# YukeWang96/QGTC_PPoPP22

Hardware: AMD Instinct MI355X
Metric: effective bit-GEMM TOPS (2*M*K*N/t), 1-bit A x 1-bit X, M=K=4096, N=64 (higher is better)
Workload: dtype fp4 (E2M1 codes of bit planes on MFMA, exact f32 sums); 1 GPU; bitMM2Bit 4096x4096x64 a=1 w=1 ob=1 (BASELINE.json configs[1], 2_7c shape); inputs=seeded Bernoulli(0.5) adjacency, uniform w-bit features, packed, resident in HBM, parallelism=replica-per-GPU x1, no data-path collective, engine=auto, issue=eager

## Files before the change

### qgtc_ppopp22_amd/csrc/bitmm_fp4_stream.hip.h

```cpp
#pragma once

namespace {

constexpr int ST_WAVES = 8;
constexpr int ST_MUL = 4;
constexpr int ST_COLS = 64;
constexpr int ST_PITCH = 68;
constexpr int ST_PIECE = 1024;
constexpr int ST_GB = 64 * ST_MUL;
constexpr int ST_STAGES = 3;

constexpr int st_pieces(int rf, int cf) { return (32 * rf / 8 + 32 * cf / 8) * (ST_GB / 128); }
constexpr int st_lds_bytes(int rf, int cf) {
    const int stages = ST_STAGES * st_pieces(rf, cf) * ST_PIECE, part = ST_MUL * 4 * rf * cf * 1024, tile = 32 * rf * ST_PITCH * 4;
    return stages > part ? (stages > tile ? stages : tile) : (part > tile ? part : tile);
}

template <int RF, int CF>
__device__ __forceinline__ constexpr int st_exp_by(int n) {
    if constexpr (RF == 2 && CF == 1) { constexpr int t[] = {5, 6, 8, 9, 11, 12, 14, 15}; return t[n]; }
    else if constexpr (RF == 2 && CF == 2) { constexpr int t[] = {4, 5, 6, 7, 8, 9, 10, 11, 12, 13, 14, 15, 16, 17, 18, 19}; return t[n]; }
    else if constexpr (RF == 4 && CF == 1) { constexpr int t[] = {4, 5, 7, 8, 9, 10, 12, 13, 14, 15, 17, 18, 19, 20, 22, 23}; return t[n]; }
    else { constexpr int t[] = {4, 4, 5, 5, 6, 7, 8, 9, 10, 10, 11, 11, 12, 13, 14, 15, 16, 16, 17, 17, 18, 19, 20, 21, 22, 22, 23, 23, 24, 25, 26, 27}; return t[n]; }
}
template <int RF, int CF>
__device__ __forceinline__ constexpr int st_shift_by(int n) {
    if constexpr (RF == 2 && CF == 1) { constexpr int t[] = {0, 0, 0, 8, 12, 12, 12, 12}; return t[n]; }
    else if constexpr (RF == 2 && CF == 2) { constexpr int t[] = {0, 0, 0, 0, 0, 2, 4, 6, 8, 10, 12, 16, 16, 16, 16, 16}; return t[n]; }
    else if constexpr (RF == 4 && CF == 1) { constexpr int t[] = {0, 0, 0, 0, 0, 0, 0, 2, 4, 8, 12, 16, 20, 20, 20, 20}; return t[n]; }
    else { constexpr int t[] = {0, 0, 0, 0, 0, 0, 0, 0, 0, 0, 0, 0, 0, 2, 4, 6, 8, 14, 16, 20, 22, 24, 24, 24, 24, 24, 24, 24, 24, 24, 24, 24}; return t[n]; }
}

template <class F, int... I>
__device__ __forceinline__ void st_for_impl(F &&f, std::integer_sequence<int, I...>) { (f(std::integral_constant<int, I>{}), ...); }
template <int N, class F>
__device__ __forceinline__ void st_for(F &&f) { st_for_impl(f, std::make_integer_sequence<int, N>{}); }

__device__ __forceinline__ void st_dma(uint32_t lds_dst, uint32_t voff, i32x4 rsrc, uint32_t soff) {
    uint32_t keep;
    asm volatile("s_mov_b32 %0, m0\n\ts_mov_b32 m0, %1\n\ts_nop 0\n\tbuffer_load_dwordx4 %2, %3, %4 offen lds\n\ts_mov_b32 m0, %0"
                 : "=&s"(keep)
                 : "s"(lds_dst), "v"(voff), "s"(rsrc), "s"(soff)
                 : "memory");
}

template <int MODE, int RF, int CF>
__global__ __launch_bounds__(64 * ST_WAVES) void k_bitmm_fp4_stream(
    const uint32_t *__restrict__ Xp, const uint32_t *__restrict__ Wp, void *__restrict__ outp, uint32_t x_bytes, uint32_t w_bytes,
    uint32_t out_bytes, int M, int K, int N, int w_lines,
    uint32_t cfg , int n_wg) {
    static_assert((RF == 2 || RF == 4) && (CF == 1 || CF == 2), "32-line fragments of a multiplying wave: left, right");
    constexpr int TR = 32 * RF, WK = ST_MUL;
    constexpr int GB = ST_GB, BPG = GB / 128, GQ = GB / 16;
    constexpr int XP = (TR / 8) * BPG, WP = (32 * CF / 8) * BPG, TOT = XP + WP;
    constexpr int FW = ST_WAVES - ST_MUL;
    static_assert(XP % FW == 0 && TOT % FW == 0, "whole rounds of the fetching waves");
    constexpr int STAGE = TOT * ST_PIECE, STAGES = ST_STAGES;
    constexpr int DMAS = TOT / FW;
    static_assert(DMAS >= 1 && DMAS <= 31, "vmcnt immediate");
    extern __shared__ __attribute__((aligned(1024))) unsigned char st_lds[];
    int (*tile)[ST_PITCH] = reinterpret_cast<int (*)[ST_PITCH]>(st_lds);
    const int tid = threadIdx.x, lane = tid & 63;
    const int wv = __builtin_amdgcn_readfirstlane(tid >> 6);
    const int fl = lane & 31, hf = lane >> 5;
#ifdef QGTC_STAMPS
    unsigned long long st_[16] = {0, 0, 0, 0, 0, 0, 0, 0, 0, 0, 0, 0, 0, 0, 0, 0};
#define ST_STAMP(i) st_[i] = __builtin_amdgcn_s_memtime()
#else
#define ST_STAMP(i) do { } while (0)
#endif
    ST_STAMP(0);
#ifdef QGTC_STAMPS
    st_[13] = __builtin_amdgcn_s_memrealtime();
#endif
    const int ob = cfg & 255u, tiles_n = static_cast<int>(cfg >> 16);
    const bool zero_skip = ((cfg >> 8) & 1u) != 0u;
    int t = static_cast<int>(blockIdx.x);
    if (tiles_n > 1) t = xcd_consecutive(t, n_wg);
    const int tm = t / tiles_n, tn = t - tm * tiles_n;
    const int m0 = tm * TR, n0 = tn * ST_COLS;
    const int kq = step128(K);
    const uint32_t row_bytes = static_cast<uint32_t>(kq) * 16u;
    const uint32_t lds0 = static_cast<uint32_t>(reinterpret_cast<uintptr_t>(st_lds));
    (void)x_bytes; (void)w_bytes; (void)out_bytes; (void)w_lines;
    const int ng = (kq + GQ - 1) / GQ;
    constexpr int NQ = RF * CF * 4;
    f32x16 acc[RF][CF];

    if (wv >= ST_MUL) {
        const int fw = wv - ST_MUL;
        const i32x4 rs_x = {static_cast<int>(reinterpret_cast<uintptr_t>(Xp)), static_cast<int>((reinterpret_cast<uintptr_t>(Xp) >> 32) & 0xffffu), static_cast<int>(x_bytes), 0x00020000};
        const i32x4 rs_w = {static_cast<int>(reinterpret_cast<uintptr_t>(Wp)), static_cast<int>((reinterpret_cast<uintptr_t>(Wp) >> 32) & 0xffffu), static_cast<int>(w_bytes), 0x00020000};
        const int rr = lane >> 3, cc = lane & 7;
        const uint32_t swz = static_cast<uint32_t>(cc ^ (rr & 6)) * 16u;
#ifdef QGTC_STREAM_TUNE
        const uint32_t voff_x = static_cast<uint32_t>(((cfg >> 9) & 1u ? 0 : m0) + rr) * row_bytes + swz, voff_w = static_cast<uint32_t>(n0 + rr) * row_bytes + swz;
        const bool no_dma = ((cfg >> 10) & 1u) != 0u;
#else
        const uint32_t voff_x = static_cast<uint32_t>(m0 + rr) * row_bytes + swz, voff_w = static_cast<uint32_t>(n0 + rr) * row_bytes + swz;
        constexpr bool no_dma = false;
#endif
        auto issue = [&](int g) {
            if (g >= ng || no_dma) return;
            const uint32_t base = lds0 + static_cast<uint32_t>(g % STAGES) * STAGE;
            const uint32_t ko = static_cast<uint32_t>(g) * GB;
#pragma unroll
            for (int j = 0; j < DMAS; j++) {
                const int p = fw + FW * j;
                if (FW * j < XP) {
                    st_dma(base + static_cast<uint32_t>(p) * ST_PIECE, voff_x, rs_x, ko + static_cast<uint32_t>(8 * (p / BPG)) * row_bytes + 128u * (p % BPG));
                } else {
                    const int pw = p - XP;
                    st_dma(base + static_cast<uint32_t>(p) * ST_PIECE, voff_w, rs_w, ko + static_cast<uint32_t>(8 * (pw / BPG)) * row_bytes + 128u * (pw % BPG));
                }
            }
        };
        issue(0);
        issue(1);
        for (int g = 0; g < ng; g++) {
            if (g + 1 < ng) asm volatile("s_waitcnt vmcnt(%0)" ::"n"(DMAS) : "memory");
            else asm volatile("s_waitcnt vmcnt(0)" ::: "memory");
#ifdef QGTC_STAMPS
            if (g == 0) ST_STAMP(1); else if (g == 5) ST_STAMP(3); else if (g == 6) ST_STAMP(7);
#endif
            __builtin_amdgcn_s_barrier();
#ifdef QGTC_STAMPS
            if (g == 0) ST_STAMP(2); else if (g == 5) ST_STAMP(4); else if (g == 6) ST_STAMP(8);
#endif
            issue(g + 2);
        }
        ST_STAMP(11);
    } else {
        const int wk = wv;
        const uint32_t frag_off = static_cast<uint32_t>(fl & 7) * 128u + static_cast<uint32_t>((4 * (wk & 1) + hf) ^ (fl & 6)) * 16u + static_cast<uint32_t>(wk >> 1) * ST_PIECE;
        const uint32_t xa0 = static_cast<uint32_t>((fl >> 3) * BPG) * ST_PIECE + frag_off;
        const uint32_t wa0 = static_cast<uint32_t>(XP + (fl >> 3) * BPG) * ST_PIECE + frag_off;
        const int my_q = 8 * (wk >> 1) + 4 * (wk & 1) + hf;
#pragma unroll
        for (int i = 0; i < RF; i++)
#pragma unroll
            for (int j = 0; j < CF; j++)
#pragma unroll
                for (int r = 0; r < 16; r++) acc[i][j][r] = 0.0f;

        auto fetch = [&](auto tail, int g, int u, u32x4 (&xr)[RF], u32x4 (&wr)[CF]) {
            const unsigned char *stage = st_lds + (g % STAGES) * STAGE;
#pragma unroll
            for (int i = 0; i < RF; i++) xr[i] = *reinterpret_cast<const u32x4 *>(stage + ((xa0 + static_cast<uint32_t>(4 * i * BPG) * ST_PIECE) ^ (32u * u)));
#pragma unroll
            for (int j = 0; j < CF; j++) wr[j] = *reinterpret_cast<const u32x4 *>(stage + ((wa0 + static_cast<uint32_t>(4 * j * BPG) * ST_PIECE) ^ (32u * u)));
            if constexpr (decltype(tail)::value) {
                if (g == ng - 1 && g * GQ + my_q + 2 * u >= kq) {
#pragma unroll
                    for (int i = 0; i < RF; i++) xr[i] = u32x4{0u, 0u, 0u, 0u};
                }
            }
        };
        constexpr int MN = 4 * RF * CF, OPB = RF + CF, EN = 4 * OPB, EP = 3;
        i32x4 A[4], B[2][CF];
        auto expand = [&](auto e_, u32x4 (&xr)[RF], u32x4 (&wr)[CF]) {
            constexpr int e = decltype(e_)::value, s = e / OPB, o = e % OPB;
            constexpr uint32_t mask = s < 3 ? 0x11111111u << s : 0x11111111u;
            constexpr bool is_a = o == 0 || o > CF;
            constexpr int f = o == 0 ? 0 : (o > CF ? o - CF : o - 1);
            u32x4 v;
            if constexpr (is_a) v = xr[f]; else v = wr[f];
            const i32x4 r = {static_cast<int>(v.x & mask), static_cast<int>(v.y & mask), static_cast<int>(v.z & mask), static_cast<int>(v.w & mask)};
            if constexpr (is_a) { A[(s * RF + f) & 3] = r; asm volatile("" : "+v"(A[(s * RF + f) & 3])); }
            else { B[s & 1][f] = r; asm volatile("" : "+v"(B[s & 1][f])); }
        };
        auto shift = [&](auto z_, u32x4 (&xr)[RF], u32x4 (&wr)[CF]) {
            constexpr int z = decltype(z_)::value, o = z >> 2, el = z & 3;
            constexpr bool is_a = o == 0 || o > CF;
            constexpr int f = o == 0 ? 0 : (o > CF ? o - CF : o - 1);
            if constexpr (is_a) { xr[f][el] >>= 3; if constexpr (el == 3) asm volatile("" : "+v"(xr[f])); }
            else { wr[f][el] >>= 3; if constexpr (el == 3) asm volatile("" : "+v"(wr[f])); }
        };
        auto any_of = [&](const u32x4 (&xr)[RF]) {
            uint32_t any = 0u;
#pragma unroll
            for (int i = 0; i < RF; i++) any |= (xr[i].x | xr[i].y) | (xr[i].z | xr[i].w);
            return any;
        };
        auto skipped = [&](uint32_t any) { return zero_skip && __ballot(any != 0u) == 0ull; };
        auto first = [&](u32x4 (&xr)[RF], u32x4 (&wr)[CF]) {
            st_for<EP>([&](auto e_) { expand(e_, xr, wr); });
        };
        auto step = [&](auto with_next, u32x4 (&xr)[RF], u32x4 (&wr)[CF], u32x4 (&nx)[RF], u32x4 (&nw)[CF], uint32_t &any_next) {
            constexpr bool NEXT = decltype(with_next)::value;
            __builtin_amdgcn_sched_barrier(0);
            st_for<MN>([&](auto n_) {
                constexpr int n = decltype(n_)::value, s = n / (RF * CF), q = n % (RF * CF);
                constexpr int i = q / CF, j = (i & 1) ? CF - 1 - q % CF : q % CF;
                constexpr int sc = s < 3 ? 128 - s : 128;
                const i32x4 a4 = A[(s * RF + i) & 3], b4 = B[s & 1][j];
                const i32x8 a8 = __builtin_shufflevector(a4, a4, 0, 1, 2, 3, -1, -1, -1, -1);
                const i32x8 b8 = __builtin_shufflevector(b4, b4, 0, 1, 2, 3, -1, -1, -1, -1);
                acc[i][j] = __builtin_amdgcn_mfma_scale_f32_32x32x64_f8f6f4(a8, b8, acc[i][j], 4, 4, 0, sc, 0, sc);
                constexpr int e0 = n == 0 ? EP : st_exp_by<RF, CF>(n == 0 ? 0 : n - 1), e1 = st_exp_by<RF, CF>(n);
                st_for<e1 - e0>([&](auto k_) {
                    constexpr int e = e0 + decltype(k_)::value;
                    if constexpr (e < EN) expand(std::integral_constant<int, e>{}, xr, wr);
                    else if constexpr (NEXT) expand(std::integral_constant<int, e - EN>{}, nx, nw);
                });
                constexpr int z0 = n == 0 ? 0 : st_shift_by<RF, CF>(n == 0 ? 0 : n - 1), z1 = st_shift_by<RF, CF>(n);
                st_for<z1 - z0>([&](auto k_) { shift(std::integral_constant<int, z0 + decltype(k_)::value>{}, xr, wr); });
                if constexpr (NEXT && n == MN - 7) {
                    any_next = any_of(nx);
                    asm volatile("" : "+v"(any_next));
                }
                __builtin_amdgcn_sched_barrier(0);
            });
        };
        using with_next = std::integral_constant<bool, true>;
        using last_step = std::integral_constant<bool, false>;
        uint32_t any_now = 0u;
        auto multiply = [&](u32x4 (&xr)[RF], u32x4 (&wr)[CF], u32x4 (&nx)[RF], u32x4 (&nw)[CF]) {
            uint32_t any_next;
            if (skipped(any_now)) {
                first(nx, nw);
                any_next = any_of(nx);
            } else {
                step(with_next{}, xr, wr, nx, nw, any_next);
            }
            any_now = any_next;
        };
        u32x4 xp[RF], wp[CF], xq[RF], wq[CF];
        using any_group = std::integral_constant<bool, true>;
        using not_last = std::integral_constant<bool, false>;
        auto trip = [&](auto tail, int g) {
            fetch(tail, g, 1, xq, wq);
            multiply(xp, wp, xq, wq);
#ifdef QGTC_STAMPS
            if (g == 5) ST_STAMP(6); else if (g == 6) ST_STAMP(10);
#endif
            asm volatile("s_waitcnt lgkmcnt(0)" ::: "memory");
            __builtin_amdgcn_s_barrier();
#ifdef QGTC_STAMPS
            if (g == 4) ST_STAMP(4); else if (g == 5) ST_STAMP(8);
#endif
            fetch(tail, g + 1, 0, xp, wp);
            multiply(xq, wq, xp, wp);
        };
        __builtin_amdgcn_s_barrier();
        ST_STAMP(2);
        fetch(any_group{}, 0, 0, xp, wp);
        first(xp, wp);
        any_now = any_of(xp);
        int g = 0;
        for (; g + 2 < ng; g++) trip(not_last{}, g);
        for (; g + 1 < ng; g++) trip(any_group{}, g);
        fetch(any_group{}, g, 1, xq, wq);
        multiply(xp, wp, xq, wq);
        if (!skipped(any_now)) step(last_step{}, xq, wq, xp, wp, any_now);
#ifdef QGTC_STAMPS
        asm volatile("" : "+v"(acc[0][0]));
#endif
        ST_STAMP(11);
    }
#ifdef QGTC_STAMPS
    st_[14] = __builtin_amdgcn_s_memrealtime();
#endif
    __syncthreads();

    constexpr int QW = NQ / ST_WAVES;
    static_assert(NQ % ST_WAVES == 0, "the quads split evenly over the waves");
    {
        f32x4 *part = reinterpret_cast<f32x4 *>(st_lds);
        if (wv < ST_MUL) {
#pragma unroll
            for (int i = 0; i < RF; i++)
#pragma unroll
                for (int j = 0; j < CF; j++)
#pragma unroll
                    for (int rq = 0; rq < 4; rq++)
                        part[(wv * NQ + (i * CF + j) * 4 + rq) * 64 + lane] = f32x4{acc[i][j][4 * rq], acc[i][j][4 * rq + 1], acc[i][j][4 * rq + 2], acc[i][j][4 * rq + 3]};
        }
        __syncthreads();
        f32x4 sum[QW];
#pragma unroll
        for (int tq = 0; tq < QW; tq++) {
            sum[tq] = part[(wv * QW + tq) * 64 + lane];
#pragma unroll
            for (int w2 = 1; w2 < WK; w2++) sum[tq] += part[(w2 * NQ + wv * QW + tq) * 64 + lane];
        }
        __syncthreads();
#pragma unroll
        for (int tq = 0; tq < QW; tq++) {
            const int q = wv * QW + tq, f = q >> 2, rq = q & 3;
            int *dst = &tile[32 * (f / CF) + 8 * rq + 4 * hf][32 * (f % CF) + fl];
#pragma unroll
            for (int e = 0; e < 4; e++) dst[e * ST_PITCH] = static_cast<int>(sum[tq][e]);
        }
        if (CF == 1) {
            for (int e = tid; e < TR * 32; e += 64 * ST_WAVES) tile[e >> 5][32 + (e & 31)] = 0;
        }
    }
    __syncthreads();
#ifdef QGTC_STAMPS
    ST_STAMP(12);
    if (lane == 0 && (blockIdx.x == 0 || blockIdx.x == 100))
        for (int i = 0; i < 16; i++) g_stamps[((blockIdx.x ? 8 : 0) + wv) * 16 + i] = st_[i];
#endif
#undef ST_STAMP

    const float maxv = __builtin_ldexpf(1.0f, ob), maxm1 = maxv - 1.0f;
    const int maxi = 1 << (ob & 31);
    const bool int_rq = ob <= 23;
    const int tiles_m = (M + TR - 1) / TR;
    const bool last_m = tm == tiles_m - 1, last_n = tn == tiles_n - 1;
    (void)last_m;

    if (MODE == 1) {
        const int col = tid >> 3, rq = tid & 7;
        const int lines = pad128(N), line_words = step128(M) * 4;
        const size_t oplane = static_cast<size_t>(lines) * line_words;
        uint32_t *out = static_cast<uint32_t *>(outp);
        const int n1 = n0 + col, word0 = m0 >> 5;
#pragma unroll
        for (int gq = 0; gq < TR / 32; gq++) {
            uint32_t q[4];
#pragma unroll
            for (int e = 0; e < 4; e++) {
                const int c = tile[32 * gq + 4 * rq + e][col];
                const int r = int_rq ? (c > maxi ? maxi - 1 : c) : requant(c, maxv, maxm1);
                q[e] = (m0 + 32 * gq + 4 * rq + e < M && n1 < N) ? static_cast<uint32_t>(r) : 0u;
            }
            uint32_t *dst = out + static_cast<size_t>(n1) * line_words + word0 + gq;
            for (int p = 0; p < ob; p++, dst += oplane) {
                const uint32_t nib = (((q[0] >> p) & 1u) << 3) | (((q[1] >> p) & 1u) << 2) | (((q[2] >> p) & 1u) << 1) | ((q[3] >> p) & 1u);
                const uint32_t wrd = or_reduce8(nib << (28u - 4u * static_cast<uint32_t>(rq)));
                if (rq == 0 && n1 < lines && word0 + gq < line_words) dst[0] = wrd;
            }
        }
        const int w_core = min(line_words, word0 + TR / 32);
        if (last_m && w_core < line_words) {
            for (int e = tid; e < ob * ST_COLS; e += 64 * ST_WAVES) {
                const int line = n0 + (e & (ST_COLS - 1)), p = e / ST_COLS;
                if (line < lines)
                    for (int wi = w_core; wi < line_words; wi++) out[p * oplane + static_cast<size_t>(line) * line_words + wi] = 0u;
            }
        }
        if (last_n && n0 + ST_COLS < lines) {
            const int nl = lines - (n0 + ST_COLS), w_end = last_m ? line_words : w_core;
            for (int e = tid; e < ob * nl; e += 64 * ST_WAVES) {
                const int line = n0 + ST_COLS + e % nl, p = e / nl;
                for (int wi = word0; wi < w_end; wi++) out[p * oplane + static_cast<size_t>(line) * line_words + wi] = 0u;
            }
        }
        return;
    }

    constexpr int QPR = ST_COLS / 4;
    const int rows_pad = pad8(M), row_words = step128(N) * 4;
    const size_t oplane = static_cast<size_t>(rows_pad) * row_words;
#pragma unroll
    for (int pass = 0; pass < TR / 32; pass++) {
        const int row = 32 * pass + tid / QPR, quad = tid % QPR;
        const i32x4 c4 = *reinterpret_cast<const i32x4 *>(&tile[row][4 * quad]);
        const int m = m0 + row, n = n0 + 4 * quad;
        if (MODE == 2) {
            if (m < M) {
                float *dst = static_cast<float *>(outp) + static_cast<size_t>(m) * N + n;
                if (n + 3 < N && (N & 3) == 0) {
                    *reinterpret_cast<f32x4 *>(dst) = f32x4{static_cast<float>(c4.x), static_cast<float>(c4.y), static_cast<float>(c4.z), static_cast<float>(c4.w)};
                } else {
#pragma unroll
                    for (int e = 0; e < 4; e++)
                        if (n + e < N) dst[e] = static_cast<float>(c4[e]);
                }
            }
            continue;
        }
        uint32_t q[4];
#pragma unroll
        for (int e = 0; e < 4; e++) {
            const int c = c4[e];
            const int r = int_rq ? (c > maxi ? maxi - 1 : c) : requant(c, maxv, maxm1);
            q[e] = (m < M && n + e < N) ? static_cast<uint32_t>(r) : 0u;
        }
        const bool store = (quad & 7) == 0 && m < rows_pad;
        const uint32_t sh_n = 28u - 4u * static_cast<uint32_t>(quad & 7);
        const int word = (n0 >> 5) + (quad >> 3);
        const int extra = (last_n && quad == QPR - 8) ? row_words - word - 1 : 0;
        uint32_t *dst = static_cast<uint32_t *>(outp) + static_cast<size_t>(m) * row_words + word;
        for (int p = 0; p < ob; p++, dst += oplane) {
            const uint32_t nib = (((q[0] >> p) & 1u) << 3) | (((q[1] >> p) & 1u) << 2) | (((q[2] >> p) & 1u) << 1) | ((q[3] >> p) & 1u);
            const uint32_t wrd = or_reduce8(nib << sh_n);
            if (store) {
                if (word < row_words) dst[0] = wrd;
                for (int x = 1; x <= extra; x++) dst[x] = 0u;
            }
        }
    }
}

}
```

Measured before the change: 738.6 TOPS.

## Pack output bit planes directly from reduced sums via ballot, skipping LDS tile

The epilogue no longer writes reduced accumulator sums into an LDS tile and re-reads them for bit-packing. For the packed-bit output mode, each wave requantizes its own sums in registers and uses wave ballots plus writelane to assemble 32-bit plane words, then stores them directly. The float output mode also writes straight from registers. This removes an LDS round trip and a block barrier from the epilogue, at the cost of a more intricate lane-to-row mapping and extra ballot instructions per bit plane.

Result: no change. 737.5 TOPS (-0.1%).

```diff
diff --git a/qgtc_ppopp22_amd/csrc/bitmm_fp4_stream.hip.h b/qgtc_ppopp22_amd/csrc/bitmm_fp4_stream.hip.h
--- a/qgtc_ppopp22_amd/csrc/bitmm_fp4_stream.hip.h
+++ b/qgtc_ppopp22_amd/csrc/bitmm_fp4_stream.hip.h
@@ -1,4 +1,6 @@
 #pragma once
+
+extern "C" __device__ int st_writelane(int value, int lane, int old) __asm("llvm.amdgcn.writelane.i32");
 
 namespace {
 
@@ -263,8 +265,9 @@
 #endif
     __syncthreads();
 
-    constexpr int QW = NQ / ST_WAVES;
-    static_assert(NQ % ST_WAVES == 0, "the quads split evenly over the waves");
+    constexpr int QW = NQ / ST_WAVES, OW = QW / CF;
+    static_assert(NQ % ST_WAVES == 0 && QW % CF == 0 && OW >= 1, "the row octets split evenly over the waves");
+    f32x4 sum[QW];
     {
         f32x4 *part = reinterpret_cast<f32x4 *>(st_lds);
         if (wv < ST_MUL) {
@@ -277,26 +280,28 @@
                         part[(wv * NQ + (i * CF + j) * 4 + rq) * 64 + lane] = f32x4{acc[i][j][4 * rq], acc[i][j][4 * rq + 1], acc[i][j][4 * rq + 2], acc[i][j][4 * rq + 3]};
         }
         __syncthreads();
-        f32x4 sum[QW];
 #pragma unroll
         for (int tq = 0; tq < QW; tq++) {
-            sum[tq] = part[(wv * QW + tq) * 64 + lane];
-#pragma unroll
-            for (int w2 = 1; w2 < WK; w2++) sum[tq] += part[(w2 * NQ + wv * QW + tq) * 64 + lane];
-        }
+            const int o = wv * OW + tq / CF, q = ((o >> 2) * CF + tq % CF) * 4 + (o & 3);
+            sum[tq] = part[q * 64 + lane];
+#pragma unroll
+            for (int w2 = 1; w2 < WK; w2++) sum[tq] += part[(w2 * NQ + q) * 64 + lane];
+        }
+    }
+    if (MODE == 1) {
         __syncthreads();
 #pragma unroll
         for (int tq = 0; tq < QW; tq++) {
-            const int q = wv * QW + tq, f = q >> 2, rq = q & 3;
-            int *dst = &tile[32 * (f / CF) + 8 * rq + 4 * hf][32 * (f % CF) + fl];
+            const int o = wv * OW + tq / CF;
+            int *dst = &tile[8 * o + 4 * hf][32 * (tq % CF) + fl];
 #pragma unroll
             for (int e = 0; e < 4; e++) dst[e * ST_PITCH] = static_cast<int>(sum[tq][e]);
         }
         if (CF == 1) {
             for (int e = tid; e < TR * 32; e += 64 * ST_WAVES) tile[e >> 5][32 + (e & 31)] = 0;
         }
-    }
-    __syncthreads();
+        __syncthreads();
+    }
 #ifdef QGTC_STAMPS
     ST_STAMP(12);
     if (lane == 0 && (blockIdx.x == 0 || blockIdx.x == 100))
@@ -351,48 +356,65 @@
         return;
     }
 
-    constexpr int QPR = ST_COLS / 4;
+    if (MODE == 2) {
+        float *out = static_cast<float *>(outp);
+#pragma unroll
+        for (int tq = 0; tq < QW; tq++) {
+            const int m = m0 + 8 * (wv * OW + tq / CF) + 4 * hf, n = n0 + 32 * (tq % CF) + fl;
+#pragma unroll
+            for (int e = 0; e < 4; e++)
+                if (m + e < M && n < N) out[static_cast<size_t>(m + e) * N + n] = sum[tq][e];
+        }
+        return;
+    }
     const int rows_pad = pad8(M), row_words = step128(N) * 4;
     const size_t oplane = static_cast<size_t>(rows_pad) * row_words;
-#pragma unroll
-    for (int pass = 0; pass < TR / 32; pass++) {
-        const int row = 32 * pass + tid / QPR, quad = tid % QPR;
-        const i32x4 c4 = *reinterpret_cast<const i32x4 *>(&tile[row][4 * quad]);
-        const int m = m0 + row, n = n0 + 4 * quad;
-        if (MODE == 2) {
-            if (m < M) {
-                float *dst = static_cast<float *>(outp) + static_cast<size_t>(m) * N + n;
-                if (n + 3 < N && (N & 3) == 0) {
-                    *reinterpret_cast<f32x4 *>(dst) = f32x4{static_cast<float>(c4.x), static_cast<float>(c4.y), static_cast<float>(c4.z), static_cast<float>(c4.w)};
-                } else {
-#pragma unroll
-                    for (int e = 0; e < 4; e++)
-                        if (n + e < N) dst[e] = static_cast<float>(c4[e]);
+    const int word0 = n0 >> 5;
+    const bool extra = last_n && row_words - word0 == 4;
+#pragma unroll
+    for (int k = 0; k < OW; k++) {
+        const int mo = m0 + 8 * (wv * OW + k);
+        uint32_t q[CF][4];
+        if (int_rq) {
+#pragma unroll
+            for (int fj = 0; fj < CF; fj++)
+#pragma unroll
+                for (int e = 0; e < 4; e++) {
+                    const int c = static_cast<int>(sum[CF * k + fj][e]);
+                    q[fj][e] = static_cast<uint32_t>(c > maxi ? maxi - 1 : c);
                 }
-            }
-            continue;
-        }
-        uint32_t q[4];
-#pragma unroll
-        for (int e = 0; e < 4; e++) {
-            const int c = c4[e];
-            const int r = int_rq ? (c > maxi ? maxi - 1 : c) : requant(c, maxv, maxm1);
-            q[e] = (m < M && n + e < N) ? static_cast<uint32_t>(r) : 0u;
-        }
-        const bool store = (quad & 7) == 0 && m < rows_pad;
-        const uint32_t sh_n = 28u - 4u * static_cast<uint32_t>(quad & 7);
-        const int word = (n0 >> 5) + (quad >> 3);
-        const int extra = (last_n && quad == QPR - 8) ? row_words - word - 1 : 0;
-        uint32_t *dst = static_cast<uint32_t *>(outp) + static_cast<size_t>(m) * row_words + word;
-        for (int p = 0; p < ob; p++, dst += oplane) {
-            const uint32_t nib = (((q[0] >> p) & 1u) << 3) | (((q[1] >> p) & 1u) << 2) | (((q[2] >> p) & 1u) << 1) | ((q[3] >> p) & 1u);
-            const uint32_t wrd = or_reduce8(nib << sh_n);
-            if (store) {
-                if (word < row_words) dst[0] = wrd;
-                for (int x = 1; x <= extra; x++) dst[x] = 0u;
-            }
-        }
-    }
-}
-
-}
+        } else {
+#pragma unroll
+            for (int fj = 0; fj < CF; fj++)
+#pragma unroll
+                for (int e = 0; e < 4; e++) q[fj][e] = static_cast<uint32_t>(requant(static_cast<int>(sum[CF * k + fj][e]), maxv, maxm1));
+        }
+#pragma unroll
+        for (int fj = 0; fj < CF; fj++)
+#pragma unroll
+            for (int e = 0; e < 4; e++) q[fj][e] = (mo + 4 * hf + e < M && n0 + 32 * fj + fl < N) ? q[fj][e] : 0u;
+        const int m = mo + (lane & 7);
+        uint32_t *dst = static_cast<uint32_t *>(outp) + static_cast<size_t>(lane >> 3) * oplane + static_cast<size_t>(m) * row_words + word0;
+        for (int p0 = 0; p0 < ob; p0 += 8, dst += 8 * oplane) {
+            int w[2] = {0, 0};
+#pragma unroll 1
+            for (int pp = 0; pp < 8 && p0 + pp < ob; pp++) {
+#pragma unroll
+                for (int fj = 0; fj < CF; fj++)
+#pragma unroll
+                    for (int e = 0; e < 4; e++) {
+                        const unsigned long long b = __ballot(((q[fj][e] >> (p0 + pp)) & 1u) != 0u);
+                        w[fj] = st_writelane(static_cast<int>(static_cast<uint32_t>(b)), 8 * pp + e, w[fj]);
+                        w[fj] = st_writelane(static_cast<int>(static_cast<uint32_t>(b >> 32)), 8 * pp + 4 + e, w[fj]);
+                    }
+            }
+            if (p0 + (lane >> 3) < ob && m < rows_pad) {
+                const uint32_t w0 = __builtin_bitreverse32(static_cast<uint32_t>(w[0])), w1 = __builtin_bitreverse32(static_cast<uint32_t>(w[1]));
+                if (extra) *reinterpret_cast<u32x4 *>(dst) = u32x4{w0, w1, 0u, 0u};
+                else *reinterpret_cast<u32x2 *>(dst) = u32x2{w0, w1};
+            }
+        }
+    }
+}
+
+}
```
